# microsoft/Tokenizer

Hardware: AMD Instinct MI355X
Metric: input MB/s encoded (cl100k_base) (higher is better)
Workload: dtype u8

## Files before the change

tokenizer_amd/csrc/tkz_api.cpp:

```cpp
#include <algorithm>
#include <cstdio>
#include <cstdlib>
#include <cstring>
#include <atomic>
#include <chrono>
#include <memory>
#include <mutex>
#include <thread>
#include <string>
#include <unordered_map>
#include <unordered_set>
#include <vector>

#include "../../include/tkz.h"
#include "tkz_adapt.h"
#include "tkz_bpe.h"
#include "tkz_corpus.h"
#include "tkz_kernels.h"
#include "tkz_pretok.h"
#include "tkz_promo_select.h"
#include "tkz_sdma.h"
#include "tkz_vocab.h"

namespace {
// ... 215 lines not shown
    int pattern = 0;
    int max_key_len = 0;
    bool pretok_seq = false;
    bool profiling = false;
    std::mutex mu;
    std::vector<Workspace*> pool;
    DevBuf t_short, t_mid, t_long, t_blob, t_pair, t_byte, t_bpair, t_bmp, t_counts3, t_memo;
    uint32_t memo_slots = 0;
    TkzTables T{};
    DevBuf t_decoff, t_decblob, t_decids;
    TkzDecodeTable D{};
    std::vector<std::pair<int32_t, std::string>> dec_vocab, dec_special;
    DevBuf t_lit;
    tkz::TkzLitTable LIT{};
    int lit_state = 0;
    bool lit_fffd = false;
    std::string lit_why;
    std::atomic<int64_t> spec_batches{0}, spec_literals{0};
    int64_t bytes_allocated = 0;
    std::atomic<int64_t> last_xcount{0}, last_xcount2{0};
    bool small_ok = false;
    bool piece_stats = false;
    int64_t latency_bytes = [] { const char* v = getenv("TKZ_LATENCY_BYTES"); return v ? (int64_t)atoll(v) : int64_t(16) << 20; }();
    bool case_equiv = false;
    size_t bmp_image_bytes = 0;
    DevBuf t_stats;
    int64_t stat_batches = 0, stat_giants = 0;
    int pending = 0;
    bool destroyed = false;
    tkz::AdaptPolicy policy;
    DevBuf t_memo_hits, t_promo;
    DevBuf t_long_log;
    int64_t long_log_n = 0;
    std::vector<DevBuf> retired;
    std::vector<tkz::KeyItem> promo_items;
    std::unordered_set<std::string> promo_keys;
    std::vector<uint32_t> promo_quads;
    uint32_t short_slots_n = 0, mid_slots_n = 0;
    std::thread promo_thread;
    std::mutex promo_join_mu;
};

namespace {

std::atomic<int> g_fork_in_flight{0};

// ... 399 lines not shown
        for (Workspace* w : e->pool) if (w != ws && w->busy) others = true;
        const AdaptPolicy::Arm arm = e->policy.may_learn(total, first && !ws->learning, c.may_learn(), e->T.memo_n != 0, e->T.max_rank < (int32_t)kPromoFlag, e->promo_items.size(), others);
        if (arm != AdaptPolicy::Arm::No && e->t_memo_hits.ensure((size_t)e->memo_slots * 4, &e->bytes_allocated) == hipSuccess &&
            e->t_long_log.ensure((size_t)kLongLogCap * kLongLogDwords * 4 + 64, &e->bytes_allocated) == hipSuccess) {
            const bool clear = arm == AdaptPolicy::Arm::YesClearMemo;
            if (!clear || (hipMemsetAsync(e->t_memo.p, 0, size_t(e->memo_slots) * sizeof(TkzMemoSlot), stream) == hipSuccess && hipStreamSynchronize(stream) == hipSuccess)) {
                ws->learn_window_start = e->policy.window_armed(clear);
                ws->learning = true;
            }
        }
        *T = e->T;
    }
    if (ws->learning) {
        T->memo_hits = e->t_memo_hits.as<uint32_t>();
        T->memo_hits_sparse = total >= (int64_t(64) << 20) ? 1u : 0u;
        if (ws->learn_window_start && first) {
            HIP_TRY(hipMemsetAsync(T->memo_hits, 0, (size_t)e->memo_slots * 4, stream));
            HIP_TRY(hipMemsetAsync(e->t_long_log.as<char>() + (size_t)kLongLogCap * kLongLogDwords * 4, 0, 64, stream));
        }
    }
    return TKZ_OK;
}

tkz::EncodeParams bind_params(Workspace* ws, const uint8_t* d_bytes, const int64_t* d_offs, int64_t n_docs, int64_t total) {
    using namespace tkz;
    char* cb = ws->w_counters.as<char>();
    EncodeParams P{};
    P.bytes = d_bytes; P.total = total; P.startbits = ws->w_startbits.as<uint64_t>(); P.docbits = ws->w_docbits.as<uint64_t>(); P.nwords = total / 64 + 1;
    P.offs = d_offs; P.n_docs = n_docs;
    P.tmp = ws->w_tmp.as<int32_t>(); P.dense = ws->w_dense.as<int32_t>(); P.tile_count = ws->w_tcount.as<int32_t>();
    P.prank = ws->w_prank.as<int32_t>(); P.prank_cap = (int64_t)(ws->w_prank.cap / 4); P.pcount = ws->w_pcount.as<int32_t>(); P.pbase = ws->w_pbase.as<int64_t>();
    P.mlist = ws->w_mlist.as<uint32_t>(); P.mquad = ws->w_mquad.as<uint4>(); P.mcap = ws->mcap; P.mcount = ws->w_mcount.as<uint32_t>();
    P.docord_base = ws->w_dbase.as<int64_t>(); P.doc_tok = ws->w_doctok.as<int32_t>(); P.counters = ws->w_counters.as<int32_t>();
    P.giant_q = ws->w_gq.as<int64_t>(); P.giant_cap = total / kArenaPiece + 1; P.giant_cnt = ws->w_gcnt.as<int32_t>();
    P.giant_count = reinterpret_cast<unsigned long long*>(cb + offsetof(CounterBlock, heavy_count));
    P.giant_ticket = reinterpret_cast<unsigned long long*>(cb + offsetof(CounterBlock, giant_ticket));
    P.heavy_flag = ws->w_heavyq.as<uint8_t>(); P.nsub = (total + kSub - 1) / kSub;
    P.pool = ws->w_pool.as<int32_t>(); P.pool_head = reinterpret_cast<unsigned long long*>(cb + offsetof(CounterBlock, pool_head)); P.pool_cap = (int64_t)(ws->w_pool.cap / 4);
    return P;
}

#ifdef TKZ_DEVPROF
unsigned long long* g_devprof = nullptr;
tkz_status devprof_arm(tkz::EncodeParams* P, hipStream_t stream) {
    { const char* ab = getenv("TKZ_DEV_ABLATE"); P->ablate = ab ? atoi(ab) : 0; }
    if (P->ablate & 16) {
// ... 73 lines not shown
                n_iso = ws->n_seg;
            }
        }
        if (!c.pretokenizes()) {
            HIP_TRY(hipMemcpyAsync(startbits, docbits, (size_t)nwords * 8, hipMemcpyDeviceToDevice, stream));
        } else if (e->pretok_seq) {
            HIP_TRY(hipMemcpyAsync(startbits, isobits, (size_t)nwords * 8, hipMemcpyDeviceToDevice, stream));
            launch_pretok_seq(L, e->pattern, d_bytes, iso_offs, n_iso, total, startbits, T.bmp_class, counters);
        } else {
            HIP_TRY(ws->w_xq.ensure((size_t)(nwords / kRowsPerWave + 4) * 16, &ws->bytes_allocated));
            launch_pretok_rows(L, e->pattern, d_bytes, iso_offs, n_iso, total, isobits, startbits, nwords, T.bmp_class, counters,
                               ws->w_xq.as<int64_t>(), reinterpret_cast<unsigned long long*>(cb + offsetof(CounterBlock, xcount)));
        }
        if (c.pretokenizes() && e->case_equiv && e->pattern == TKZ_PATTERN_CL100K) launch_case_equiv_fix(L, d_bytes, total, isobits, startbits);
        if (special) launch_lit_fix(L, startbits, isobits, ws->w_specbits.as<uint64_t>(), ws->w_endbits.as<uint64_t>(), nwords);
    }
    if (c.bitmap_only()) {
        HIP_TRY(hipMemcpyAsync(c.d_bitmap, startbits, (size_t)nwords * 8, hipMemcpyDeviceToDevice, stream));
    } else {
        EncodeParams P = bind_params(ws, d_bytes, d_offs, n_docs, total);
        P.lane_piece = kLanePiece;
        P.latency = total <= e->latency_bytes ? 1 : 0;
        P.tc_atomic = (L.side || P.latency) ? 1 : 0;
        if (L.side && nsample < 0) ++ws->forked_batches;
        P.coop_cap = total / P.lane_piece + 64;
        P.coop_q = ws->w_coopq.as<uint64_t>();
        P.coop_count = reinterpret_cast<unsigned long long*>(cb + offsetof(CounterBlock, coop_count));
        P.coop_ticket = reinterpret_cast<unsigned long long*>(cb + offsetof(CounterBlock, coop_ticket));
        P.lq_cnt = ws->w_lqcnt.as<int32_t>(); P.lq_base = ws->w_lqbase.as<int64_t>(); P.lq = ws->w_lq.as<uint64_t>(); P.lq_cap = total / (kShortMax + 1) + 64;
        P.lq_total = reinterpret_cast<int64_t*>(cb + offsetof(CounterBlock, lq_total)); P.lq_bsum = ws->w_bsum.as<int64_t>();
        P.miss_sums = reinterpret_cast<unsigned long long*>(cb + offsetof(CounterBlock, miss_short));
        P.stats = e->piece_stats ? e->t_stats.as<unsigned long long>() : nullptr;
        if (P.stats) HIP_TRY(hipMemcpyAsync(e->t_stats.as<char>() + 64, P.stats, 64, hipMemcpyDeviceToDevice, stream));
        P.place128 = ws->place128 ? 1 : 0;
        P.promo = T.promo; P.pextra = T.promo ? ws->w_pextra.as<int32_t>() : nullptr;
        if (ws->learning) {
            P.long_log = e->t_long_log.as<uint32_t>(); P.long_log_cap = (int32_t)kLongLogCap; P.long_log_sparse = T.memo_hits_sparse ? 1 : 0;
            P.long_log_count = reinterpret_cast<unsigned long long*>(e->t_long_log.as<char>() + (size_t)kLongLogCap * kLongLogDwords * 4);
        }
        if (special) { P.specbits = ws->w_specbits.as<uint64_t>(); P.lit_meta = e->LIT.meta; P.lit_blob = e->LIT.blob; P.n_lit = e->LIT.n; P.lit_repl = c.d_repl; }
        TKZ_TRY(devprof_arm(&P, stream));
        int64_t* ndocstarts = reinterpret_cast<int64_t*>(cb + offsetof(CounterBlock, ndocstarts));
        int64_t* npieces = reinterpret_cast<int64_t*>(cb + offsetof(CounterBlock, npieces));
        int64_t* grand = reinterpret_cast<int64_t*>(cb + offsetof(CounterBlock, grand));
        const uint64_t* markbits = po ? startbits : docbits;
        P.docbits = markbits;
// ... 1615 lines not shown
```

tokenizer_amd/csrc/tkz_kernels.h:

```cpp
#pragma once
#include <stdint.h>

#include "tkz_simt.h"
#include "tkz_tables.h"

namespace tkz {

constexpr int kThreads = 256;
constexpr int kSub = 1024;
constexpr int kHalo = 64;
constexpr int kShortMax = 16;
#ifndef TKZ_MERGE_GROUP
#define TKZ_MERGE_GROUP 16
#endif
constexpr int kMergeGroup = TKZ_MERGE_GROUP;
constexpr int kDenseCap = 256 * kMergeGroup;
#ifndef TKZ_ARENA_DWORDS
#define TKZ_ARENA_DWORDS 2560
#endif
constexpr int kArenaDwords = TKZ_ARENA_DWORDS;
constexpr int kArenaPiece = 1024;
#ifndef TKZ_LANE_PIECE
#define TKZ_LANE_PIECE 128
#endif
// ... 26 lines not shown
    const int64_t* pbase;
    uint32_t* mlist; int32_t mcap;
    uint4* mquad;
    uint32_t* mcount;
    const int64_t* docord_base;
    int32_t* doc_tok;
    int32_t* counters;
    int32_t latency;
    int32_t lane_piece;
    uint8_t* heavy_flag; int64_t nsub;
    int32_t* pool; unsigned long long* pool_head; int64_t pool_cap;
    int64_t* giant_q; unsigned long long* giant_count; int64_t giant_cap; int32_t* giant_cnt;
    unsigned long long* giant_ticket;
    uint64_t* coop_q; unsigned long long* coop_count; unsigned long long* coop_ticket; int64_t coop_cap;
    int32_t* lq_cnt; int64_t* lq_base; int64_t* lq_total; int64_t* lq_bsum; uint64_t* lq; int64_t lq_cap;
    unsigned long long* miss_sums;
    unsigned long long* devprof;
    int32_t ablate;
    unsigned long long* stats;
    uint32_t* long_log; unsigned long long* long_log_count; int32_t long_log_cap; int32_t long_log_sparse;
    int32_t* pextra;
    const uint4* promo;
    int32_t tc_atomic;
    int32_t place128;
    const uint64_t* specbits; const uint32_t* lit_meta; const uint8_t* lit_blob; int32_t n_lit;
    const uint64_t* lit_repl;
};

constexpr int kLitMax = 256, kLitMaxLen = 128, kLitFffdHead = 8, kLitMetaHead = 16;
struct TkzLitTable { const uint32_t* meta; const uint8_t* blob; int32_t n; int32_t blob_bytes; };
struct TkzLitAllowed { uint64_t m[kLitMax / 64]; };

constexpr int kSmallLdsBytesNeeded = 86 * 1024;
constexpr int kSmallMaxBytes = 131072, kSmallMaxBytesO200k = 65536, kSmallMaxDocs = 8192, kSmallMaxDoc = 1024;
struct SmallArgs {
    const uint8_t* h_bytes; const int64_t* h_offs;
    int32_t* out; int64_t out_cap; int64_t* out_offs;
    int64_t* h_result;
    uint64_t* docbits; uint64_t* startbits;
    int32_t* pcount; int64_t* pbase; int64_t* docord_base; int64_t* tile_base;
    int32_t counter_words;
    int64_t* counts3[2];
};

typedef void (*KernelHook)(void* ctx, int kernel_id, int phase , hipStream_t s);
struct Launch { hipStream_t stream; KernelHook hook; void* hook_ctx; hipStream_t side = nullptr, side2 = nullptr; hipEvent_t ev_fork = nullptr, ev_join = nullptr, ev_join2 = nullptr; };
// ... 56 lines not shown
```

tokenizer_amd/csrc/tkz_kernels.hip:

```cpp
#include "tkz_kernels.h"

#include <type_traits>

#include "tkz_bpe.h"
#include "tkz_classes.h"
#include "tkz_corpus.h"
#include "tkz_pretok.h"
#include "tkz_simt.h"

namespace tkz {

TKZ_KERNEL(256) void k_docmark(const int64_t* offs, int64_t n_items, int64_t total, uint64_t* bits, int32_t* counters) {
    const int64_t stride = simt::nblocks() * simt::nthreads();
    for (int64_t d = simt::bid() * simt::nthreads() + simt::tid(); d <= n_items; d += stride) {
        const int64_t pos = offs[d];
        bool ok = pos >= 0 && pos <= total;
        if (d == 0) ok = ok && pos == 0;
        if (d == n_items) ok = ok && pos == total;
        else ok = ok && pos <= offs[d + 1];
        if (!ok) { simt::atomic_or((unsigned*)&counters[0], (unsigned)kErrOffsets); continue; }
        const int64_t w = pos >> 6;
        if (d > 0) { const int64_t prev = offs[d - 1]; if (prev >= 0 && prev <= pos && (prev >> 6) == w) continue; }
        uint64_t m = 1ull << (pos & 63);
        int64_t cur = pos;
// ... 827 lines not shown
            const int64_t p = a0 + 4 * i;
            if (p + 4 <= total) w[i] = *reinterpret_cast<const uint32_t*>(bytes + p);
            else { w[i] = 0; for (int j = 0; j < 4; ++j) if (p + j < total) w[i] |= (uint32_t)bytes[p + j] << (8 * j); }
        }
    }
#pragma unroll
    for (int i = 0; i < 4; ++i) pw[i] = simt::alignbit(w[i + 1], w[i], sh);
}

TKZ_HD uint32_t tkz_result_entry(bool dense, int cnt, int off) { return kMrDone | (dense ? kMrDense : 0u) | ((uint32_t)(cnt - 1) << kMrCntShift) | (uint32_t)off; }
TKZ_HD uint32_t tkz_result_inline(int cnt) { return kMrDone | kMrInline | ((uint32_t)(cnt - 1) << kMrCntShift); }
TKZ_HD int tkz_result_cnt(uint32_t r) { return (int)((r >> kMrCntShift) & 1023u) + 1; }
TKZ_HD int tkz_result_off(uint32_t r) { return (int)(r & kMrOffMask); }

template <int N, class Pre>
TKZ_DEV int tkz_find_list(const Pre* pre, int g) {
    int q = 0;
#pragma unroll
    for (int step = N / 2; step >= 1; step >>= 1) if (pre[q + step] <= g) q += step;
    return q;
}

constexpr int kMsStride = TkzBpeGeom<16>::kStride, kMsIdStride = TkzBpeGeom<16>::kIdStride;
#ifndef TKZ_MS_SHORT_LEN
#define TKZ_MS_SHORT_LEN 8
#endif
#ifndef TKZ_MS_TWO_MIN
#define TKZ_MS_TWO_MIN 320
#endif
constexpr int kMsTwoListsMin = TKZ_MS_TWO_MIN;
constexpr int kMsShortLen = TKZ_MS_SHORT_LEN;
struct MsLds { uint4* pr; uint32_t* ids; uint16_t* rec; uint16_t* idx; int* extra; uint16_t* pre; const uint16_t* brank16; };
constexpr int kMsLdsBytes = kMsStride * 64 * 4 + kMsIdStride * 64 * 4 + 2 * (2 * 64 + 2 * 64) + 4 * kGroup + 2 * (kGroup + 1);
constexpr int kMsLdsQuads = (kMsLdsBytes + 15) / 16;
static_assert((kMsThreads / 64) * kMsLdsQuads * 16 + 512 <= 40960, "k_merge_short: four workgroups a CU (160 KB of LDS, allocated in units of 1,280 bytes)");
TKZ_DEV MsLds tkz_ms_lds(uint4* wave_quads, const uint16_t* brank16) {
    MsLds L;
    uint8_t* b = reinterpret_cast<uint8_t*>(wave_quads);
    L.pr = reinterpret_cast<uint4*>(b); b += kMsStride * 64 * 4;
    L.ids = reinterpret_cast<uint32_t*>(b); b += kMsIdStride * 64 * 4;
    L.extra = reinterpret_cast<int*>(b); b += 4 * kGroup;
    L.rec = reinterpret_cast<uint16_t*>(b); b += 2 * 2 * 64;
    L.idx = reinterpret_cast<uint16_t*>(b); b += 2 * 2 * 64;
    L.pre = reinterpret_cast<uint16_t*>(b);
    L.brank16 = brank16;
    return L;
}
TKZ_DEV void tkz_ms_brank_init(const TkzTables& T, uint16_t* s_brank16) {
    for (int i = simt::tid(); i < 256; i += simt::nthreads()) {
        const uint32_t v = (uint32_t)T.byte_rank[i];
        s_brank16[i] = (uint16_t)(v >= (uint32_t)TKZ_PSEUDO_BASE ? 0xFFFFu : (v < 0xFFFEu ? v : 0xFFFEu));
    }
}
TKZ_DEV void tkz_merge_short_group(const TkzTables& T, const EncodeParams& P, int64_t grp, const MsLds& LD) {
    constexpr int NMAX = 16, STRIDE = kMsStride, IDSTRIDE = kMsIdStride;
    static_assert(kGroup == 16 && kShortMax == 16, "list entries: 4 bits of sub-tile, 10 of index; 10 of relpos, 4 of length, 1 flag");
    const int lane = simt::lane();
    const uint16_t* s_brank16 = LD.brank16;
    auto byte_id = [&](uint32_t b) -> uint32_t {
        const uint32_t v = s_brank16[b];
        return v < 0xFFFEu ? v : (v == 0xFFFFu ? (uint32_t)TKZ_PSEUDO_BASE + b : (uint32_t)T.byte_rank[b]);
    };
    auto pair_rank = [&](uint32_t b0, uint32_t b1) -> int32_t { return T.bytepair_rank[(b0 << 8) | b1]; };
    const int64_t sub0 = grp * kGroup;
    if (sub0 >= P.nsub) return;
    uint16_t* s_rec = LD.rec;
    uint16_t* s_idx = LD.idx;
    int* s_extra = LD.extra;
    uint16_t* s_pre = LD.pre;
    uint32_t* ids = LD.ids + lane * IDSTRIDE;
    uint32_t* pr = reinterpret_cast<uint32_t*>(LD.pr) + lane * STRIDE;
    int my_np = 0, my_ns = 0;
    if (lane < kGroup && sub0 + lane < P.nsub) { my_np = P.pcount[sub0 + lane]; my_ns = (int)(P.mcount[sub0 + lane] & 0xFFFFu); }
    { const int nl_ = lane < kGroup && sub0 + lane < P.nsub ? (int)(P.mcount[sub0 + lane] >> 16) : 0; if (my_ns + nl_ > P.mcap) my_ns = 0; }
    int ntotal;
    { const int pre = tkz_wave_scan_sum(my_ns, &ntotal); if (lane <= kGroup) s_pre[lane] = (uint16_t)pre; }
    if (lane < kGroup) s_extra[lane] = 0;
    uint32_t* const ml0 = P.mlist + sub0 * (int64_t)P.mcap;
    int err = 0, dused = 0, done = 0;
    int nl0 = 0, nl1 = 0;
    int st_look = 0, st_hit = 0;
    int32_t* const dense = P.dense + grp * kDenseCap;
    const bool memo = T.memo_n != 0;
    const bool sparse = T.memo_hits_sparse != 0;
    const bool count_hits = T.memo_hits != nullptr && (!sparse || (grp & 7) == 0);
    auto assign = [&](bool have, int cnt, int si, int j, int rel) -> int32_t* {
        int btot;
        const bool big = have && cnt > 4;
        const int doff = dused + tkz_wave_scan_sum(big ? cnt : 0, &btot);
        int32_t* dst = nullptr;
        if (have) {
            if (!big) ml0[si * (int64_t)P.mcap + j] = tkz_result_inline(cnt);
            else {
                const bool packed = doff + cnt <= kDenseCap;
                dst = packed ? dense + doff : P.tmp + ((sub0 + si) * kSub + rel);
                ml0[si * (int64_t)P.mcap + j] = tkz_result_entry(packed, cnt, packed ? doff : rel);
            }
            if (cnt > 1) simt::atomic_add(&s_extra[si], cnt - 1);
        }
        dused += btot;
        return dst;
    };
    uint4* const mq0 = P.mquad + sub0 * (int64_t)P.mcap;
    auto key_of = [&](uint4 kq, int len, uint32_t* kw, bool* nul) {
        kw[0] = kq.x; kw[1] = kq.y; kw[2] = kq.z; kw[3] = kq.w;
        uint32_t z = 0;
#pragma unroll
        for (int i = 0; i < 4; ++i) {
            const int nb = len - 4 * i;
            const uint32_t m = nb >= 4 ? 0xFFFFFFFFu : (nb <= 0 ? 0u : ((1u << (8 * nb)) - 1u));
            z |= (kw[i] - 0x01010101u) & ~kw[i] & 0x80808080u & m;
        }
        *nul = z != 0;
    };
    auto memo_phase = [&](int take, uint32_t r16, uint32_t ix, uint4 fkq) -> bool {
        (void)simt::ballot(true);
        const bool mine = lane < take;
        const int si = (int)(ix >> 10), j = (int)(ix & 1023u), rel = (int)(r16 & 1023u), len = (int)((r16 >> 10) & 15u) + 1;
        bool hit = false;
        uint32_t hit_slot = 0;
        uint4 vv; vv.x = vv.y = vv.z = vv.w = 0;
        if (mine && memo) {
            uint32_t kw[4];
            bool nul;
            key_of(fkq, len, kw, &nul);
            const uint32_t b = tkz_mulhi(tkz_hash_memo(kw, (uint32_t)len), T.memo_n / kMemoWays) * kMemoWays;
#pragma unroll
            for (int wy = 0; wy < (int)kMemoWays; ++wy) {
                const TkzMemoSlot* slot = &T.memo[b + wy];
                const uint4 kk = tkz_load16(&slot->k[0]);
                const uint4 v = tkz_load16(&slot->v[0]);
                const bool h = !nul && ((v.x & v.y & v.z & v.w) & kMemoValid) && v.x != kMemoBusy && kk.x == kw[0] && kk.y == kw[1] && kk.z == kw[2] && kk.w == kw[3] &&
                               ((v.y >> 27) & 15u) == (uint32_t)(len - 1);
                if (h) { hit = true; vv = v; hit_slot = b + wy; }
            }
        }
        if (count_hits) {
            if (hit && (!sparse || lane == ((done * 5 + nl0 + nl1) & 63)) && tkz_atomic_load_agent(&T.memo_hits[hit_slot]) < kMemoHitsSat)
                simt::atomic_add(reinterpret_cast<int*>(&T.memo_hits[hit_slot]), 1);
        }
        if (P.stats) { st_look += tkz_popc64(simt::ballot(mine && memo)); st_hit += tkz_popc64(simt::ballot(hit)); }
        const int cnt = hit ? (int)((vv.x >> 29) & 3u) + 1 : 0;
        (void)assign(hit, cnt, si, j, rel);
        if (hit) {
            uint4 tq; tq.x = vv.x & 0x07FFFFFFu; tq.y = vv.y & 0x07FFFFFFu; tq.z = vv.z & 0x07FFFFFFu; tq.w = vv.w & 0x07FFFFFFu;
            mq0[si * (int64_t)P.mcap + j] = tq;
        }
        (void)simt::ballot(true);
        return mine && !hit;
    };
    auto run_batch = [&](int c, int n) {
        (void)simt::ballot(true);
        int cnt = 0, si = 0, j = 0, rel = 0, e1 = 0, len = 1;
        bool nul = false;
        uint32_t alive = 1;
        uint32_t kw[4] = {0, 0, 0, 0};
        if (lane < n) {
            const uint32_t r16 = s_rec[64 * c + lane], ix = s_idx[64 * c + lane];
            si = (int)(ix >> 10); j = (int)(ix & 1023u); rel = (int)(r16 & 1023u); len = (int)((r16 >> 10) & 15u) + 1;
            key_of(tkz_load16(&mq0[si * (int64_t)P.mcap + j]), len, kw, &nul);
            cnt = tkz_bpe_lane_f<NMAX>(T, kw, len, ids, pr, byte_id, pair_rank, &alive, &e1);
            err |= e1;
        }
        int32_t* dst = assign(lane < n, cnt, si, j, rel);
        if (lane < n) {
            uint32_t t4[4] = {0, 0, 0, 0};
            int i = 0;
            for (uint32_t a = alive; a; a &= a - 1) { const uint32_t t = ids[tkz_ctz32(a)]; if (dst) dst[i] = (int32_t)t; if (i < 4) { if (i == 0) t4[0] = t; else if (i == 1) t4[1] = t; else if (i == 2) t4[2] = t; else t4[3] = t; } ++i; }
            if (cnt <= 4) { uint4 tq; tq.x = t4[0]; tq.y = t4[1]; tq.z = t4[2]; tq.w = t4[3]; mq0[si * (int64_t)P.mcap + j] = tq; }
            if (memo && cnt <= 4 && !e1 && !nul) {
                const uint32_t b = tkz_mulhi(tkz_hash_memo(kw, (uint32_t)len), T.memo_n / kMemoWays) * kMemoWays;
                bool placed = false;
#pragma unroll
                for (int wy = 0; wy < (int)kMemoWays; ++wy) {
                    TkzMemoSlot* slot = &T.memo[b + wy];
                    if (!placed && *reinterpret_cast<volatile uint32_t*>(&slot->v[0]) == 0u && simt::atomic_cas(&slot->v[0], 0u, kMemoBusy) == 0u) {
                        uint4 kk; kk.x = kw[0]; kk.y = kw[1]; kk.z = kw[2]; kk.w = kw[3];
                        *reinterpret_cast<uint4*>(&slot->k[0]) = kk;
                        uint4 nv; nv.x = kMemoValid | ((uint32_t)(cnt - 1) << 29) | t4[0]; nv.y = kMemoValid | ((uint32_t)(len - 1) << 27) | t4[1]; nv.z = kMemoValid | t4[2]; nv.w = kMemoValid | t4[3];
                        *reinterpret_cast<uint4*>(&slot->v[0]) = nv;
                        placed = true;
                    }
                }
            }
        }
        (void)simt::ballot(true);
    };
    (void)simt::ballot(true);
    auto request = [&](int g, uint32_t* r16, uint32_t* ix, uint4* kq) {
        *r16 = 0; *ix = 0; kq->x = kq->y = kq->z = kq->w = 0;
        if (g < ntotal) {
            const int q = tkz_find_list<kGroup>(s_pre, g), j = g - (int)s_pre[q];
            const uint32_t ent = tkz_load_nt(&ml0[q * (int64_t)P.mcap + j]);
            *kq = tkz_load16(&mq0[q * (int64_t)P.mcap + j]);
            *r16 = (ent & 1023u) | (((ent >> kMrLenShift) & 15u) << 10);
            *ix = (uint32_t)((q << 10) | j);
        }
    };
    const bool two = ntotal >= kMsTwoListsMin;
    uint32_t a_r16, a_ix;
    uint4 a_kq;
    request(lane, &a_r16, &a_ix, &a_kq);
    while (done < ntotal) {
        const int take = ntotal - done < 64 ? ntotal - done : 64;
        const uint32_t f_r16 = a_r16, f_ix = a_ix;
        const uint4 f_kq = a_kq;
        done += take;
        request(done + lane, &a_r16, &a_ix, &a_kq);
        const bool merge_it = memo_phase(take, f_r16, f_ix, f_kq);
        const int cls = two && ((f_r16 >> 10) & 15u) >= (uint32_t)kMsShortLen ? 1 : 0;
#pragma unroll 1
        for (int c = 0; c < 2; ++c) {
            const uint64_t m = simt::ballot(merge_it && cls == c);
            const int had = c ? nl1 : nl0;
            const int pos = had + tkz_popc64(m & tkz_lowmask(lane)), tot = had + tkz_popc64(m);
            const bool here = merge_it && cls == c;
            if (here && pos < 64) { s_rec[64 * c + pos] = (uint16_t)f_r16; s_idx[64 * c + pos] = (uint16_t)f_ix; }
            if (tot >= 64) {
                run_batch(c, 64);
                if (here && pos >= 64) { s_rec[64 * c + pos - 64] = (uint16_t)f_r16; s_idx[64 * c + pos - 64] = (uint16_t)f_ix; }
                if (c) nl1 = tot - 64; else nl0 = tot - 64;
            } else if (c) nl1 = tot; else nl0 = tot;
        }
    }
    if (nl0 + nl1 <= 64 && nl1 > 0) {
        (void)simt::ballot(true);
        if (lane < nl1) { s_rec[nl0 + lane] = s_rec[64 + lane]; s_idx[nl0 + lane] = s_idx[64 + lane]; }
        nl0 += nl1; nl1 = 0;
    }
#pragma unroll 1
    for (int c = 0; c < 2; ++c) { const int n = c ? nl1 : nl0; if (n > 0) run_batch(c, n); }
    (void)simt::ballot(true);
    if (lane < kGroup && sub0 + lane < P.nsub) {
        const int tc = my_np + s_extra[lane] + (P.pextra ? P.pextra[sub0 + lane] : 0);
        if (P.tc_atomic) simt::atomic_add(&P.tile_count[sub0 + lane], tc);
        else P.tile_count[sub0 + lane] = tc;
    }
    if (err) simt::atomic_or((unsigned*)&P.counters[0], (unsigned)err);
    if (P.stats && lane == 0 && st_look) { simt::atomic_add64(&P.stats[0], (unsigned long long)st_look); simt::atomic_add64(&P.stats[1], (unsigned long long)st_hit); }
}
TKZ_DEV bool tkz_attempt_failed(const EncodeParams& P) { return (P.counters[0] & (kErrMissCap | kErrCapacity)) != 0; }

TKZ_KERNEL_OCC(kMsThreads, 4) void k_merge_short(TkzTables T, EncodeParams P) {
    if (tkz_attempt_failed(P)) return;
    TKZ_SHARED uint4 s_wave[kMsThreads / 64][kMsLdsQuads];
    TKZ_SHARED uint16_t s_brank16[256];
    tkz_ms_brank_init(T, s_brank16);
    simt::sync();
    const int64_t grp = tkz_xcd_block(simt::bid(), simt::nblocks()) * (kMsThreads / 64) + simt::wave();
    tkz_merge_short_group(T, P, grp, tkz_ms_lds(s_wave[simt::wave()], s_brank16));
}

#ifndef TKZ_LONG_PARTS
#define TKZ_LONG_PARTS 4
#endif
#ifndef TKZ_LONG_DENSE
#define TKZ_LONG_DENSE 192
#endif
constexpr int kLongParts = TKZ_LONG_PARTS, kLongDense = TKZ_LONG_DENSE;
static_assert(kLongParts >= 1 && kLongParts <= 64 && 64 % kLongParts == 0, "a part is a whole number of the chunk's 64 sub-tiles");
constexpr int kLongSeg = 384;
constexpr int kFastPiece = 64;
static_assert(kFastPiece <= kLanePiece && kFastPiece <= kSmallLanePiece, "every caller's lane limit covers the fast batches");
constexpr int kLenClasses = 16;
TKZ_HD int tkz_len_class(int len) {
    if (len <= 32) return (len - 17) >> 2;
    if (len <= 64) return 4 + ((len - 33) >> 3);
    if (len <= 128) return len <= 96 ? 8 : 9;
    if (len <= 256) return len <= 192 ? 10 : 11;
    if (len <= 512) return len <= 384 ? 12 : 13;
    return len <= 768 ? 14 : 15;
}
struct LongLds { uint32_t* arena; int arena_dwords; int* pre; int* cls; uint16_t* ord; int32_t* brank; };
// ... 454 lines not shown
            if (cnt > 1) simt::atomic_add(&P.tile_count[sub], cnt - 1);
        }
        simt::sync();
    }
    if (err) simt::atomic_or((unsigned*)&P.counters[0], (unsigned)err);
}
TKZ_KERNEL(64) void k_merge_coop(TkzTables T, EncodeParams P) {
    if (tkz_attempt_failed(P)) return;
    TKZ_SHARED uint4 s_lds[kCoopLdsQuads];
    tkz_merge_coop_queue(T, P, s_lds, (unsigned long long)simt::bid(), (unsigned long long)simt::nblocks());
}

constexpr int kMergeLatWaveQuads = kMsLdsQuads > kLongLdsQuads ? kMsLdsQuads : kLongLdsQuads;
template <bool COMPACT>
TKZ_KERNEL_OCC(kMsThreads, 3) void k_merge_latency(TkzTables T, EncodeParams P, int nb_short, int nb_long) {
    if (tkz_attempt_failed(P)) return;
    TKZ_SHARED uint4 s_wave[kMsThreads / 64][kMergeLatWaveQuads];
    TKZ_SHARED uint16_t s_brank16[256];
    const int b = (int)simt::bid();
    if (b < nb_short) {
        tkz_ms_brank_init(T, s_brank16);
        simt::sync();
        const int64_t grp = tkz_xcd_block(b, nb_short) * (kMsThreads / 64) + simt::wave();
        tkz_merge_short_group(T, P, grp, tkz_ms_lds(s_wave[simt::wave()], s_brank16));
    } else {
        const LongLds LD = tkz_long_lds(s_wave[simt::wave()]);
        tkz_long_brank_init(T, LD.brank);
        tkz_merge_long_chunks<COMPACT, kLongPartsLatency, -1>(T, P, (int64_t)(b - nb_short) * (kMsThreads / 64) + simt::wave(), (int64_t)nb_long * (kMsThreads / 64), LD, P.lane_piece);
    }
}

#ifndef TKZ_PLACE_OCC
#define TKZ_PLACE_OCC 7
#endif
constexpr int kPlacePer = 4;
constexpr int kPlaceBig = 8;
#ifndef TKZ_PLACE_FAST_BIG
#define TKZ_PLACE_FAST_BIG 64
#endif
constexpr int kPlaceFastBig = TKZ_PLACE_FAST_BIG;
constexpr int kStageMin = 64 * kPlaceBig + 16;
#ifndef TKZ_PLACE_STAGE
#define TKZ_PLACE_STAGE 784
#endif
constexpr int kStageBatch = TKZ_PLACE_STAGE;
static_assert(kStageBatch >= kStageMin && kStageBatch % 16 == 0, "whole quads, and room for one batch of the general path");
template <int SLOTS, int STAGE> constexpr int kPlaceLdsQuadsT = STAGE / 4 + SLOTS + SLOTS / 4 + 1 + SLOTS / 4;
// ... 1308 lines not shown
    {
        uint4* s_kmask = s_raw + nwaves * kProbeLdsQuads;
        tkz_probe_kmask_init(s_kmask);
        simt::sync();
        for (int sub = wave; sub < nsub; sub += nwaves) {
            ProbeText tx;
            tkz_probe_request_text(P, sub, &tx);
            tkz_probe_subtile<true>(T, P, sub, tkz_probe_lds(s_raw + wave * kProbeLdsQuads, s_kmask), tx, -1);
            (void)simt::ballot(true);
        }
    }
    simt::sync();
    if (tid == 0) { int f = P.counters[0] != 0; for (int t = 0; t < nsub; ++t) f |= (P.heavy_flag[t] & 2u) != 0; s_flag = f; }
    simt::sync();
    if (s_flag) {
        if (tid == 0) { A.h_result[0] = 1; A.h_result[1] = P.counters[0]; }
        return;
    }
    stamp();
    {
        uint16_t* s_brank16 = reinterpret_cast<uint16_t*>(s_raw + 8 * kMsLdsQuads);
        tkz_ms_brank_init(T, s_brank16);
        simt::sync();
        for (int g = wave; g < 8 && g * kGroup < nsub; g += nwaves) tkz_merge_short_group(T, P, g, tkz_ms_lds(s_raw + wave * kMsLdsQuads, s_brank16));
    }
    simt::sync();
    stamp();
    if (wave == 0) {
        const LongLds LD = tkz_long_lds(s_raw);
        tkz_long_brank_init(T, LD.brank);
        if (T.max_rank <= kVarCompactMaxRank) tkz_merge_long_chunks<true>(T, P, 0, 1, LD, kSmallLanePiece);
        else tkz_merge_long_chunks<false>(T, P, 0, 1, LD, kSmallLanePiece);
    }
    simt::sync();
    stamp();
    if (wave == 0) {
        int carry = 0;
        for (int q0 = 0; q0 < nsub; q0 += 64) {
            const int q = q0 + lane;
            int tot;
            const int pre = carry + tkz_wave_scan_sum(q < nsub ? P.tile_count[q] : 0, &tot);
            if (q < nsub) A.tile_base[q] = pre;
            carry += tot;
        }
        if (lane == 0) { A.h_result[2] = carry; A.tile_base[nsub] = carry; }
    }
    simt::sync();
// ... 74 lines not shown
static void launch_long_queue(const Launch& L, const EncodeParams& P, int64_t nsub) {
    const int64_t nchunks = cdiv(nsub, 64), g4 = cdiv(nchunks, 4);
    TKZ_LAUNCH(k_long_count, g4 < 4096 ? g4 : 4096, kThreads, L.stream, P);
    launch_scan2(L, nchunks * kLenClasses, P.lq_bsum, P.lq_cnt, P.lq_base, P.lq_total, 1, nullptr, nullptr, nullptr, 1, -1);
    TKZ_LAUNCH(k_long_scatter, g4 < 4096 ? g4 : 4096, kThreads, L.stream, P);
}
static void launch_long_q(hipStream_t st, const TkzTables& T, const EncodeParams& P, int64_t cap) {
    const int64_t ranges = cdiv(P.lq_cap, kLqRangeLong), grid = ranges < cap ? (ranges < 1 ? 1 : ranges) : cap;
    if (T.max_rank <= kVarCompactMaxRank) TKZ_LAUNCH((k_merge_long_q<true>), grid, 64, st, T, P);
    else TKZ_LAUNCH((k_merge_long_q<false>), grid, 64, st, T, P);
}
static void launch_coop(hipStream_t st, const TkzTables& T, const EncodeParams& P, int64_t grid, int64_t cap) {
    TKZ_LAUNCH(k_merge_coop, grid < cap ? grid : cap, 64, st, T, P);
}
constexpr int64_t kSideLongGrid = 2048, kSideCoopGrid = 1024;
void launch_encode(const Launch& L, const TkzTables& T, const EncodeParams& P, int64_t nsub) {
    hook(L, K_ENCODE, 0);
    if (P.specbits) TKZ_LAUNCH(k_probe_special, xcd_grid(cdiv(nsub, (kThreads / 64) * kProbePer)), kThreads, L.stream, T, P);
    else TKZ_LAUNCH(k_probe, xcd_grid(cdiv(nsub, (kThreads / 64) * kProbePer)), kThreads, L.stream, T, P);
    hook(L, K_ENCODE, 1);
    { const int64_t g = grid_for(nsub); TKZ_LAUNCH(k_list_stats, g < 1024 ? g : 1024, kThreads, L.stream, (const uint32_t*)P.mcount, nsub, P.mcap, P.counters,
                                                     (const uint8_t*)P.heavy_flag, P.startbits, P.nwords, P.total, P.giant_q, P.giant_count, P.giant_cap,
                                                     (const uint32_t*)P.mlist, P.coop_q, P.coop_count, P.coop_cap, (int)P.lane_piece, P.miss_sums); }
    const int64_t nb_short = xcd_grid(cdiv(nsub, (kMsThreads / 64) * kGroup));
    if (P.latency) {
        hook(L, K_HEAVY, 0);
        launch_giants(L, T, P);
        hook(L, K_HEAVY, 1);
        const int64_t chunks = cdiv(nsub, 64) * kLongPartsLatency, nb_long = cdiv(chunks < 65536 ? chunks : 65536, kMsThreads / 64);
        hook(L, K_MERGE_SHORT, 0);
        if (T.max_rank <= kVarCompactMaxRank) TKZ_LAUNCH((k_merge_latency<true>), nb_short + nb_long, kMsThreads, L.stream, T, P, (int)nb_short, (int)nb_long);
        else TKZ_LAUNCH((k_merge_latency<false>), nb_short + nb_long, kMsThreads, L.stream, T, P, (int)nb_short, (int)nb_long);
        launch_coop(L.stream, T, P, 512, kCoopGrid);
        hook(L, K_MERGE_SHORT, 1);
    } else if (!L.side) {
        hook(L, K_MERGE_SHORT, 0);
        TKZ_LAUNCH(k_merge_short, nb_short, kMsThreads, L.stream, T, P);
        hook(L, K_MERGE_SHORT, 1);
        hook(L, K_HEAVY, 0);
        launch_giants(L, T, P);
        launch_long_queue(L, P, nsub);
        launch_long_q(L.stream, T, P, kLongQGrid);
        launch_coop(L.stream, T, P, cdiv(nsub, 64), kCoopGrid);
        hook(L, K_HEAVY, 1);
    } else {
        hook(L, K_HEAVY, 0);
        launch_giants(L, T, P);
// ... 149 lines not shown
```

Before: 271,100.

## Let each merge-short wave process a run of consecutive groups with shared batches

Generalizes the short-piece merge so one wave can handle a run of R consecutive groups. Pending BPE batches are carried across group boundaries by packing a group index into each list entry, and dense offsets and tile counts are tracked per group. The aim is fewer partially filled 64-lane batches and less per-wave setup. The default run length is 1 and can be raised through TKZ_MS_RUN, and the new fold and dense-offset logic adds extra ballots and LDS round-trips per batch.

```diff
diff --git a/tokenizer_amd/csrc/tkz_api.cpp b/tokenizer_amd/csrc/tkz_api.cpp
--- a/tokenizer_amd/csrc/tkz_api.cpp
+++ b/tokenizer_amd/csrc/tkz_api.cpp
@@ -261,6 +261,8 @@
     bool small_ok = false;
     bool piece_stats = false;
     int64_t latency_bytes = [] { const char* v = getenv("TKZ_LATENCY_BYTES"); return v ? (int64_t)atoll(v) : int64_t(16) << 20; }();
+    int ms_run_forced = [] { const char* v = getenv("TKZ_MS_RUN"); const int n = v ? atoi(v) : 0; return n >= 1 && n <= 16 ? n : 0; }();
+    int ms_two_min = [] { const char* v = getenv("TKZ_MS_TWO_MIN"); const int n = v ? atoi(v) : 0; return n > 0 ? n : 0; }();
     bool case_equiv = false;
     size_t bmp_image_bytes = 0;
     DevBuf t_stats;
@@ -706,6 +708,7 @@
     return TKZ_OK;
 }
 
+constexpr int kMsRunAuto = 1;
 tkz::EncodeParams bind_params(Workspace* ws, const uint8_t* d_bytes, const int64_t* d_offs, int64_t n_docs, int64_t total) {
     using namespace tkz;
     char* cb = ws->w_counters.as<char>();
@@ -825,6 +828,7 @@
         P.lane_piece = kLanePiece;
         P.latency = total <= e->latency_bytes ? 1 : 0;
         P.tc_atomic = (L.side || P.latency) ? 1 : 0;
+        P.ms_run = e->ms_run_forced ? e->ms_run_forced : kMsRunAuto; P.ms_two_min = e->ms_two_min;
         if (L.side && nsample < 0) ++ws->forked_batches;
         P.coop_cap = total / P.lane_piece + 64;
         P.coop_q = ws->w_coopq.as<uint64_t>();
diff --git a/tokenizer_amd/csrc/tkz_kernels.h b/tokenizer_amd/csrc/tkz_kernels.h
--- a/tokenizer_amd/csrc/tkz_kernels.h
+++ b/tokenizer_amd/csrc/tkz_kernels.h
@@ -72,6 +72,8 @@
     int32_t* pextra;
     const uint4* promo;
     int32_t tc_atomic;
+    int32_t ms_run;
+    int32_t ms_two_min;
     int32_t place128;
     const uint64_t* specbits; const uint32_t* lit_meta; const uint8_t* lit_blob; int32_t n_lit;
     const uint64_t* lit_repl;
diff --git a/tokenizer_amd/csrc/tkz_kernels.hip b/tokenizer_amd/csrc/tkz_kernels.hip
--- a/tokenizer_amd/csrc/tkz_kernels.hip
+++ b/tokenizer_amd/csrc/tkz_kernels.hip
@@ -873,6 +873,8 @@
 }
 
 constexpr int kMsStride = TkzBpeGeom<16>::kStride, kMsIdStride = TkzBpeGeom<16>::kIdStride;
+constexpr int kMsRunMax = 16;
+constexpr int kMsRunRegs = kMsRunMax * kGroup / 64;
 #ifndef TKZ_MS_SHORT_LEN
 #define TKZ_MS_SHORT_LEN 8
 #endif
@@ -881,18 +883,17 @@
 #endif
 constexpr int kMsTwoListsMin = TKZ_MS_TWO_MIN;
 constexpr int kMsShortLen = TKZ_MS_SHORT_LEN;
-struct MsLds { uint4* pr; uint32_t* ids; uint16_t* rec; uint16_t* idx; int* extra; uint16_t* pre; const uint16_t* brank16; };
-constexpr int kMsLdsBytes = kMsStride * 64 * 4 + kMsIdStride * 64 * 4 + 2 * (2 * 64 + 2 * 64) + 4 * kGroup + 2 * (kGroup + 1);
+struct MsLds { uint4* pr; uint32_t* ids; uint32_t* ent; uint16_t* pre; const uint16_t* brank16; };
+constexpr int kMsLdsBytes = kMsStride * 64 * 4 + kMsIdStride * 64 * 4 + 4 * (2 * 64) + 2 * (kGroup + 1);
 constexpr int kMsLdsQuads = (kMsLdsBytes + 15) / 16;
 static_assert((kMsThreads / 64) * kMsLdsQuads * 16 + 512 <= 40960, "k_merge_short: four workgroups a CU (160 KB of LDS, allocated in units of 1,280 bytes)");
+static_assert(kMsRunMax * kGroup * 4 <= kMsStride * 64 * 4 && kMsRunMax <= 16 && kMsRunMax <= 64, "the fold's counters fit the pr arena; a list entry has 4 bits for the group");
 TKZ_DEV MsLds tkz_ms_lds(uint4* wave_quads, const uint16_t* brank16) {
     MsLds L;
     uint8_t* b = reinterpret_cast<uint8_t*>(wave_quads);
     L.pr = reinterpret_cast<uint4*>(b); b += kMsStride * 64 * 4;
     L.ids = reinterpret_cast<uint32_t*>(b); b += kMsIdStride * 64 * 4;
-    L.extra = reinterpret_cast<int*>(b); b += 4 * kGroup;
-    L.rec = reinterpret_cast<uint16_t*>(b); b += 2 * 2 * 64;
-    L.idx = reinterpret_cast<uint16_t*>(b); b += 2 * 2 * 64;
+    L.ent = reinterpret_cast<uint32_t*>(b); b += 4 * 2 * 64;
     L.pre = reinterpret_cast<uint16_t*>(b);
     L.brank16 = brank16;
     return L;
@@ -903,9 +904,23 @@
         s_brank16[i] = (uint16_t)(v >= (uint32_t)TKZ_PSEUDO_BASE ? 0xFFFFu : (v < 0xFFFEu ? v : 0xFFFEu));
     }
 }
-TKZ_DEV void tkz_merge_short_group(const TkzTables& T, const EncodeParams& P, int64_t grp, const MsLds& LD) {
+TKZ_DEV void tkz_ms_wave_fence() {
+#ifndef TKZ_HOSTEMU
+    __builtin_amdgcn_fence(__ATOMIC_ACQ_REL, "wavefront");
+    __builtin_amdgcn_wave_barrier();
+#endif
+    (void)simt::ballot(true);
+}
+TKZ_DEV int tkz_ms_read_lane(int v, int src) {
+#ifndef TKZ_HOSTEMU
+    return __builtin_amdgcn_readlane(v, __builtin_amdgcn_readfirstlane(src));
+#else
+    return simt::shfl(v, src);
+#endif
+}
+TKZ_DEV void tkz_merge_short_run(const TkzTables& T, const EncodeParams& P, int64_t grp0, int R, const MsLds& LD) {
     constexpr int NMAX = 16, STRIDE = kMsStride, IDSTRIDE = kMsIdStride;
-    static_assert(kGroup == 16 && kShortMax == 16, "list entries: 4 bits of sub-tile, 10 of index; 10 of relpos, 4 of length, 1 flag");
+    static_assert(kGroup == 16 && kShortMax == 16, "list entries: 10 bits of relpos, 4 of length; 10 of index, 4 of sub-tile; 4 of group");
     const int lane = simt::lane();
     const uint16_t* s_brank16 = LD.brank16;
     auto byte_id = [&](uint32_t b) -> uint32_t {
@@ -913,46 +928,89 @@
         return v < 0xFFFEu ? v : (v == 0xFFFFu ? (uint32_t)TKZ_PSEUDO_BASE + b : (uint32_t)T.byte_rank[b]);
     };
     auto pair_rank = [&](uint32_t b0, uint32_t b1) -> int32_t { return T.bytepair_rank[(b0 << 8) | b1]; };
-    const int64_t sub0 = grp * kGroup;
-    if (sub0 >= P.nsub) return;
-    uint16_t* s_rec = LD.rec;
-    uint16_t* s_idx = LD.idx;
-    int* s_extra = LD.extra;
+    const int64_t rsub0 = grp0 * kGroup;
+    if (rsub0 >= P.nsub) return;
+    const int nrun = (int)(P.nsub - rsub0 < (int64_t)R * kGroup ? P.nsub - rsub0 : (int64_t)R * kGroup);
+    uint32_t* s_ent = LD.ent;
     uint16_t* s_pre = LD.pre;
+    int* s_fold = reinterpret_cast<int*>(LD.pr);
     uint32_t* ids = LD.ids + lane * IDSTRIDE;
     uint32_t* pr = reinterpret_cast<uint32_t*>(LD.pr) + lane * STRIDE;
-    int my_np = 0, my_ns = 0;
-    if (lane < kGroup && sub0 + lane < P.nsub) { my_np = P.pcount[sub0 + lane]; my_ns = (int)(P.mcount[sub0 + lane] & 0xFFFFu); }
-    { const int nl_ = lane < kGroup && sub0 + lane < P.nsub ? (int)(P.mcount[sub0 + lane] >> 16) : 0; if (my_ns + nl_ > P.mcap) my_ns = 0; }
-    int ntotal;
-    { const int pre = tkz_wave_scan_sum(my_ns, &ntotal); if (lane <= kGroup) s_pre[lane] = (uint16_t)pre; }
-    if (lane < kGroup) s_extra[lane] = 0;
-    uint32_t* const ml0 = P.mlist + sub0 * (int64_t)P.mcap;
-    int err = 0, dused = 0, done = 0;
+    int ns_k[kMsRunRegs], ex_k[kMsRunRegs];
+    int nrun_entries = 0;
+#pragma unroll
+    for (int k = 0; k < kMsRunRegs; ++k) {
+        ns_k[k] = 0; ex_k[k] = 0;
+        if (k * 64 < nrun) {
+            if (k * 64 + lane < nrun) {
+                const uint32_t mc = P.mcount[rsub0 + k * 64 + lane];
+                ex_k[k] = P.pcount[rsub0 + k * 64 + lane] + (P.pextra ? P.pextra[rsub0 + k * 64 + lane] : 0);
+                ns_k[k] = (int)(mc & 0xFFFFu);
+                if (ns_k[k] + (int)(mc >> 16) > P.mcap) ns_k[k] = 0;
+            }
+            int t;
+            (void)tkz_wave_scan_sum(ns_k[k], &t);
+            nrun_entries += t;
+        }
+    }
+    int g = 0, ntotal = 0, done = 0, nl_in = 0;
+    int64_t grp = grp0, sub0 = rsub0;
+    uint32_t* ml0 = P.mlist + sub0 * (int64_t)P.mcap;
+    uint4* mq0 = P.mquad + sub0 * (int64_t)P.mcap;
+    int err = 0;
+    int dused = 0;
     int nl0 = 0, nl1 = 0;
     int st_look = 0, st_hit = 0;
-    int32_t* const dense = P.dense + grp * kDenseCap;
     const bool memo = T.memo_n != 0;
     const bool sparse = T.memo_hits_sparse != 0;
-    const bool count_hits = T.memo_hits != nullptr && (!sparse || (grp & 7) == 0);
-    auto assign = [&](bool have, int cnt, int si, int j, int rel) -> int32_t* {
+    bool count_hits = false;
+    auto assign = [&](bool have, int cnt, int ge, int si, int j, int rel) -> int32_t* {
         int btot;
         const bool big = have && cnt > 4;
-        const int doff = dused + tkz_wave_scan_sum(big ? cnt : 0, &btot);
+        const int pre = tkz_wave_scan_sum(big ? cnt : 0, &btot);
+        int doff = 0;
+        const int ge0 = simt::first_lane(ge);
+        if (btot > 0 && simt::ballot(ge != ge0) == 0) {
+            doff = tkz_ms_read_lane(dused, ge0) + pre;
+            if (lane == ge0) dused = dused + btot < kDenseCap ? dused + btot : kDenseCap;
+        } else if (btot > 0) {
+            const int gprev = simt::shfl_up(ge, 1);
+            const uint64_t heads = simt::ballot(lane == 0 || ge != gprev);
+            const int h = tkz_msb64((heads & tkz_lowmask(lane + 1)) | 1ull);
+            doff = simt::shfl(dused, ge) + pre - simt::shfl(pre, h);
+            for (uint64_t hm = heads; hm; hm &= hm - 1) {
+                const int h0 = tkz_ctz64(hm);
+                const uint64_t rest = hm & (hm - 1);
+                const int hg = tkz_ms_read_lane(ge, h0);
+                const int end = rest ? tkz_ms_read_lane(pre, tkz_ctz64(rest)) : btot;
+                const int tot = end - tkz_ms_read_lane(pre, h0);
+                if (lane == hg) dused = dused + tot < kDenseCap ? dused + tot : kDenseCap;
+            }
+        }
+        const int64_t s = rsub0 + ge * kGroup + si;
         int32_t* dst = nullptr;
         if (have) {
-            if (!big) ml0[si * (int64_t)P.mcap + j] = tkz_result_inline(cnt);
+            uint32_t* const ans = P.mlist + s * (int64_t)P.mcap + j;
+            if (!big) *ans = tkz_result_inline(cnt);
             else {
                 const bool packed = doff + cnt <= kDenseCap;
-                dst = packed ? dense + doff : P.tmp + ((sub0 + si) * kSub + rel);
-                ml0[si * (int64_t)P.mcap + j] = tkz_result_entry(packed, cnt, packed ? doff : rel);
-            }
-            if (cnt > 1) simt::atomic_add(&s_extra[si], cnt - 1);
-        }
-        dused += btot;
+                dst = packed ? P.dense + (grp0 + ge) * kDenseCap + doff : P.tmp + (s * kSub + rel);
+                *ans = tkz_result_entry(packed, cnt, packed ? doff : rel);
+            }
+        }
+        const bool add = have && cnt > 1;
+        if (simt::ballot(add)) {
+#pragma unroll
+            for (int k = 0; k < kMsRunRegs; ++k) if (k * 64 < nrun) s_fold[k * 64 + lane] = 0;
+            tkz_ms_wave_fence();
+            if (add) simt::atomic_add(&s_fold[ge * kGroup + si], cnt - 1);
+            tkz_ms_wave_fence();
+#pragma unroll
+            for (int k = 0; k < kMsRunRegs; ++k) if (k * 64 < nrun) ex_k[k] += s_fold[k * 64 + lane];
+            tkz_ms_wave_fence();
+        }
         return dst;
     };
-    uint4* const mq0 = P.mquad + sub0 * (int64_t)P.mcap;
     auto key_of = [&](uint4 kq, int len, uint32_t* kw, bool* nul) {
         kw[0] = kq.x; kw[1] = kq.y; kw[2] = kq.z; kw[3] = kq.w;
         uint32_t z = 0;
@@ -987,12 +1045,12 @@
             }
         }
         if (count_hits) {
-            if (hit && (!sparse || lane == ((done * 5 + nl0 + nl1) & 63)) && tkz_atomic_load_agent(&T.memo_hits[hit_slot]) < kMemoHitsSat)
+            if (hit && (!sparse || lane == ((done * 5 + nl0 + nl1 - nl_in) & 63)) && tkz_atomic_load_agent(&T.memo_hits[hit_slot]) < kMemoHitsSat)
                 simt::atomic_add(reinterpret_cast<int*>(&T.memo_hits[hit_slot]), 1);
         }
         if (P.stats) { st_look += tkz_popc64(simt::ballot(mine && memo)); st_hit += tkz_popc64(simt::ballot(hit)); }
         const int cnt = hit ? (int)((vv.x >> 29) & 3u) + 1 : 0;
-        (void)assign(hit, cnt, si, j, rel);
+        (void)assign(hit, cnt, g, si, j, rel);
         if (hit) {
             uint4 tq; tq.x = vv.x & 0x07FFFFFFu; tq.y = vv.y & 0x07FFFFFFu; tq.z = vv.z & 0x07FFFFFFu; tq.w = vv.w & 0x07FFFFFFu;
             mq0[si * (int64_t)P.mcap + j] = tq;
@@ -1006,19 +1064,23 @@
         bool nul = false;
         uint32_t alive = 1;
         uint32_t kw[4] = {0, 0, 0, 0};
+        const uint32_t ent = s_ent[64 * c + (lane < n ? lane : n - 1)];
+        const int ge = (int)(ent >> 28);
+        uint4* quad = nullptr;
         if (lane < n) {
-            const uint32_t r16 = s_rec[64 * c + lane], ix = s_idx[64 * c + lane];
-            si = (int)(ix >> 10); j = (int)(ix & 1023u); rel = (int)(r16 & 1023u); len = (int)((r16 >> 10) & 15u) + 1;
-            key_of(tkz_load16(&mq0[si * (int64_t)P.mcap + j]), len, kw, &nul);
+            si = (int)((ent >> 24) & 15u); j = (int)((ent >> 14) & 1023u); rel = (int)(ent & 1023u); len = (int)((ent >> 10) & 15u) + 1;
+            quad = P.mquad + (rsub0 + ge * kGroup + si) * (int64_t)P.mcap + j;
+            key_of(tkz_load16(quad), len, kw, &nul);
             cnt = tkz_bpe_lane_f<NMAX>(T, kw, len, ids, pr, byte_id, pair_rank, &alive, &e1);
             err |= e1;
         }
-        int32_t* dst = assign(lane < n, cnt, si, j, rel);
+        tkz_ms_wave_fence();
+        int32_t* dst = assign(lane < n, cnt, ge, si, j, rel);
         if (lane < n) {
             uint32_t t4[4] = {0, 0, 0, 0};
             int i = 0;
             for (uint32_t a = alive; a; a &= a - 1) { const uint32_t t = ids[tkz_ctz32(a)]; if (dst) dst[i] = (int32_t)t; if (i < 4) { if (i == 0) t4[0] = t; else if (i == 1) t4[1] = t; else if (i == 2) t4[2] = t; else t4[3] = t; } ++i; }
-            if (cnt <= 4) { uint4 tq; tq.x = t4[0]; tq.y = t4[1]; tq.z = t4[2]; tq.w = t4[3]; mq0[si * (int64_t)P.mcap + j] = tq; }
+            if (cnt <= 4) { uint4 tq; tq.x = t4[0]; tq.y = t4[1]; tq.z = t4[2]; tq.w = t4[3]; *quad = tq; }
             if (memo && cnt <= 4 && !e1 && !nul) {
                 const uint32_t b = tkz_mulhi(tkz_hash_memo(kw, (uint32_t)len), T.memo_n / kMemoWays) * kMemoWays;
                 bool placed = false;
@@ -1037,60 +1099,95 @@
         }
         (void)simt::ballot(true);
     };
-    (void)simt::ballot(true);
-    auto request = [&](int g, uint32_t* r16, uint32_t* ix, uint4* kq) {
+    auto request = [&](int x, uint32_t* r16, uint32_t* ix, uint4* kq) {
         *r16 = 0; *ix = 0; kq->x = kq->y = kq->z = kq->w = 0;
-        if (g < ntotal) {
-            const int q = tkz_find_list<kGroup>(s_pre, g), j = g - (int)s_pre[q];
+        if (x < ntotal) {
+            const int q = tkz_find_list<kGroup>(s_pre, x), j = x - (int)s_pre[q];
             const uint32_t ent = tkz_load_nt(&ml0[q * (int64_t)P.mcap + j]);
             *kq = tkz_load16(&mq0[q * (int64_t)P.mcap + j]);
             *r16 = (ent & 1023u) | (((ent >> kMrLenShift) & 15u) << 10);
             *ix = (uint32_t)((q << 10) | j);
         }
     };
-    const bool two = ntotal >= kMsTwoListsMin;
-    uint32_t a_r16, a_ix;
-    uint4 a_kq;
-    request(lane, &a_r16, &a_ix, &a_kq);
-    while (done < ntotal) {
-        const int take = ntotal - done < 64 ? ntotal - done : 64;
-        const uint32_t f_r16 = a_r16, f_ix = a_ix;
-        const uint4 f_kq = a_kq;
-        done += take;
-        request(done + lane, &a_r16, &a_ix, &a_kq);
-        const bool merge_it = memo_phase(take, f_r16, f_ix, f_kq);
-        const int cls = two && ((f_r16 >> 10) & 15u) >= (uint32_t)kMsShortLen ? 1 : 0;
+    const bool two = nrun_entries >= (P.ms_two_min > 0 ? P.ms_two_min : kMsTwoListsMin);
+    for (g = 0; g < R; ++g) {
+        grp = grp0 + g; sub0 = grp * kGroup;
+        if (sub0 >= P.nsub) break;
+        ml0 = P.mlist + sub0 * (int64_t)P.mcap;
+        mq0 = P.mquad + sub0 * (int64_t)P.mcap;
+        count_hits = T.memo_hits != nullptr && (!sparse || (grp & 7) == 0);
+        int my_ns = 0;
+        {
+            int v = ns_k[0];
+#pragma unroll
+            for (int k = 1; k < kMsRunRegs; ++k) if ((g >> 2) == k) v = ns_k[k];
+            v = simt::shfl(v, ((g & 3) << 4) | (lane & 15));
+            if (lane < kGroup) my_ns = v;
+        }
+        (void)simt::ballot(true);
+        { const int pre = tkz_wave_scan_sum(my_ns, &ntotal); if (lane <= kGroup) s_pre[lane] = (uint16_t)pre; }
+        tkz_ms_wave_fence();
+        done = 0; nl_in = nl0 + nl1;
+        uint32_t a_r16, a_ix;
+        uint4 a_kq;
+        request(lane, &a_r16, &a_ix, &a_kq);
+        while (done < ntotal) {
+            const int take = ntotal - done < 64 ? ntotal - done : 64;
+            const uint32_t f_r16 = a_r16, f_ix = a_ix;
+            const uint4 f_kq = a_kq;
+            done += take;
+            request(done + lane, &a_r16, &a_ix, &a_kq);
+            const bool merge_it = memo_phase(take, f_r16, f_ix, f_kq);
+            const int cls = two && ((f_r16 >> 10) & 15u) >= (uint32_t)kMsShortLen ? 1 : 0;
+            const uint32_t f_ent = f_r16 | (f_ix << 14) | ((uint32_t)g << 28);
 #pragma unroll 1
-        for (int c = 0; c < 2; ++c) {
-            const uint64_t m = simt::ballot(merge_it && cls == c);
-            const int had = c ? nl1 : nl0;
-            const int pos = had + tkz_popc64(m & tkz_lowmask(lane)), tot = had + tkz_popc64(m);
-            const bool here = merge_it && cls == c;
-            if (here && pos < 64) { s_rec[64 * c + pos] = (uint16_t)f_r16; s_idx[64 * c + pos] = (uint16_t)f_ix; }
-            if (tot >= 64) {
-                run_batch(c, 64);
-                if (here && pos >= 64) { s_rec[64 * c + pos - 64] = (uint16_t)f_r16; s_idx[64 * c + pos - 64] = (uint16_t)f_ix; }
-                if (c) nl1 = tot - 64; else nl0 = tot - 64;
-            } else if (c) nl1 = tot; else nl0 = tot;
+            for (int c = 0; c < 2; ++c) {
+                const uint64_t m = simt::ballot(merge_it && cls == c);
+                const int had = c ? nl1 : nl0;
+                const int pos = had + tkz_popc64(m & tkz_lowmask(lane)), tot = had + tkz_popc64(m);
+                const bool here = merge_it && cls == c;
+                if (here && pos < 64) s_ent[64 * c + pos] = f_ent;
+                if (tot >= 64) {
+                    run_batch(c, 64);
+                    if (here && pos >= 64) s_ent[64 * c + pos - 64] = f_ent;
+                    if (c) nl1 = tot - 64; else nl0 = tot - 64;
+                } else if (c) nl1 = tot; else nl0 = tot;
+            }
         }
     }
     if (nl0 + nl1 <= 64 && nl1 > 0) {
-        (void)simt::ballot(true);
-        if (lane < nl1) { s_rec[nl0 + lane] = s_rec[64 + lane]; s_idx[nl0 + lane] = s_idx[64 + lane]; }
+        tkz_ms_wave_fence();
+        uint32_t mine = 0xFFFFFFFFu;
+        if (lane < nl0) mine = s_ent[lane]; else if (lane < nl0 + nl1) mine = s_ent[64 + lane - nl0];
+        const int key = (int)(mine >> 28);
+        int rank = 0;
+        for (int q = 0; q < R; ++q) {
+            const uint64_t m = simt::ballot(lane < nl0 + nl1 && key == q);
+            if (lane < nl0 + nl1 && key == q) rank += tkz_popc64(m & tkz_lowmask(lane));
+            else if (key > q) rank += tkz_popc64(m);
+        }
+        tkz_ms_wave_fence();
+        if (lane < nl0 + nl1) s_ent[rank] = mine;
         nl0 += nl1; nl1 = 0;
     }
 #pragma unroll 1
     for (int c = 0; c < 2; ++c) { const int n = c ? nl1 : nl0; if (n > 0) run_batch(c, n); }
     (void)simt::ballot(true);
-    if (lane < kGroup && sub0 + lane < P.nsub) {
-        const int tc = my_np + s_extra[lane] + (P.pextra ? P.pextra[sub0 + lane] : 0);
-        if (P.tc_atomic) simt::atomic_add(&P.tile_count[sub0 + lane], tc);
-        else P.tile_count[sub0 + lane] = tc;
+#pragma unroll
+    for (int k = 0; k < kMsRunRegs; ++k) {
+        if (k * 64 + lane < nrun) {
+            const int64_t sub = rsub0 + k * 64 + lane;
+            const int tc = ex_k[k];
+            if (P.tc_atomic) simt::atomic_add(&P.tile_count[sub], tc);
+            else P.tile_count[sub] = tc;
+        }
     }
     if (err) simt::atomic_or((unsigned*)&P.counters[0], (unsigned)err);
     if (P.stats && lane == 0 && st_look) { simt::atomic_add64(&P.stats[0], (unsigned long long)st_look); simt::atomic_add64(&P.stats[1], (unsigned long long)st_hit); }
 }
 TKZ_DEV bool tkz_attempt_failed(const EncodeParams& P) { return (P.counters[0] & (kErrMissCap | kErrCapacity)) != 0; }
+
+TKZ_HD int tkz_ms_run(const EncodeParams& P) { return P.ms_run < 1 ? 1 : (P.ms_run > kMsRunMax ? kMsRunMax : P.ms_run); }
 
 TKZ_KERNEL_OCC(kMsThreads, 4) void k_merge_short(TkzTables T, EncodeParams P) {
     if (tkz_attempt_failed(P)) return;
@@ -1098,8 +1195,9 @@
     TKZ_SHARED uint16_t s_brank16[256];
     tkz_ms_brank_init(T, s_brank16);
     simt::sync();
-    const int64_t grp = tkz_xcd_block(simt::bid(), simt::nblocks()) * (kMsThreads / 64) + simt::wave();
-    tkz_merge_short_group(T, P, grp, tkz_ms_lds(s_wave[simt::wave()], s_brank16));
+    const int R = tkz_ms_run(P);
+    const int64_t run = tkz_xcd_block(simt::bid(), simt::nblocks()) * (kMsThreads / 64) + simt::wave();
+    tkz_merge_short_run(T, P, run * R, R, tkz_ms_lds(s_wave[simt::wave()], s_brank16));
 }
 
 #ifndef TKZ_LONG_PARTS
@@ -1600,7 +1698,7 @@
         tkz_ms_brank_init(T, s_brank16);
         simt::sync();
         const int64_t grp = tkz_xcd_block(b, nb_short) * (kMsThreads / 64) + simt::wave();
-        tkz_merge_short_group(T, P, grp, tkz_ms_lds(s_wave[simt::wave()], s_brank16));
+        tkz_merge_short_run(T, P, grp, 1, tkz_ms_lds(s_wave[simt::wave()], s_brank16));
     } else {
         const LongLds LD = tkz_long_lds(s_wave[simt::wave()]);
         tkz_long_brank_init(T, LD.brank);
@@ -2955,7 +3053,7 @@
         uint16_t* s_brank16 = reinterpret_cast<uint16_t*>(s_raw + 8 * kMsLdsQuads);
         tkz_ms_brank_init(T, s_brank16);
         simt::sync();
-        for (int g = wave; g < 8 && g * kGroup < nsub; g += nwaves) tkz_merge_short_group(T, P, g, tkz_ms_lds(s_raw + wave * kMsLdsQuads, s_brank16));
+        for (int g = wave; g < 8 && g * kGroup < nsub; g += nwaves) tkz_merge_short_run(T, P, g, 1, tkz_ms_lds(s_raw + wave * kMsLdsQuads, s_brank16));
     }
     simt::sync();
     stamp();
@@ -3076,7 +3174,7 @@
     { const int64_t g = grid_for(nsub); TKZ_LAUNCH(k_list_stats, g < 1024 ? g : 1024, kThreads, L.stream, (const uint32_t*)P.mcount, nsub, P.mcap, P.counters,
                                                      (const uint8_t*)P.heavy_flag, P.startbits, P.nwords, P.total, P.giant_q, P.giant_count, P.giant_cap,
                                                      (const uint32_t*)P.mlist, P.coop_q, P.coop_count, P.coop_cap, (int)P.lane_piece, P.miss_sums); }
-    const int64_t nb_short = xcd_grid(cdiv(nsub, (kMsThreads / 64) * kGroup));
+    const int64_t nb_short = xcd_grid(cdiv(nsub, (int64_t)(kMsThreads / 64) * kGroup * (P.latency ? 1 : tkz_ms_run(P))));
     if (P.latency) {
         hook(L, K_HEAVY, 0);
         launch_giants(L, T, P);
```

After: 271,000. Within noise of the previous version (-0.0%).
